# pmeletis/IV2019-boosting-semantic-segmentation-with-weak-labels

Hardware: NVIDIA B200
Metric: train_images_per_s (higher is better)
Workload: dtype bf16

## Files before the change

iv2019-boosting-semantic-segmentation-with-weak-labels_b200/csrc/conv_igemm_sm100.cu:

```cuda
#include <cuda.h>

#include <cstdlib>
#include <map>
#include <mutex>
#include <tuple>
#include <vector>

#include "common.cuh"
#include "tc_sm100.cuh"

namespace wlseg {

int check_conv_params(const wlseg_conv_params* p);
int conv_fprop_direct(const wlseg_conv_params* p, const void* x, const void* w, void* y, const float* scale,
                      const float* shift, const void* residual, cudaStream_t s);

constexpr int kBM = 128;
constexpr int kBK = 64;
constexpr int kUmmaK = 16;
constexpr int kEpiWarp0 = 4;
constexpr int kABytes = kBM * kBK * 2;
constexpr int kSmemBudget = 224 * 1024;

struct IgemmParams {
// ... 195 lines not shown
            const uint32_t lbar = mapa_shared(bar, 0);
            tma_load_4d_pair(a_dst, &prm.map_a, lbar, cc * kBK, q0 * prm.stride - prm.pad_left + s * prm.dilation,
                             p0 * prm.stride - prm.pad_top + r * prm.dilation, n);
            tma_load_3d_pair(b_dst, &prm.map_b, lbar, cc * kBK, tap, k0 + (int)rank * Cfg::kBRows);
          } else {
            mbar_arrive_expect_tx(bar, Cfg::kStageBytes);
            tma_load_4d(a_dst, &prm.map_a, bar, cc * kBK, q0 * prm.stride - prm.pad_left + s * prm.dilation,
                        p0 * prm.stride - prm.pad_top + r * prm.dilation, n);
            tma_load_3d(b_dst, &prm.map_b, bar, cc * kBK, tap, k0);
          }
          if (++stage == stages) { stage = 0; phase ^= 1; }
          if (++cc == prm.cchunks) {
            cc = 0; ++tap;
            if (++s == prm.S) { s = 0; ++r; }
          }
        }
      }
    }
  } else if (warp == 1) {
    if (kHalo && lane == 0) {
      constexpr uint32_t idesc = make_idesc(kBM, BN);
      mbar_wait(smem_u32(bfull_bar), 0);
      int iter = 0;
      for (int tile = unit0; tile < prm.units; tile += unit_step, ++iter) {
        const int acc = iter & 1, ab = iter & 1;
        const uint32_t ph = (iter >> 1) & 1;
        mbar_wait(smem_u32(tempty_bar + acc), ph ^ 1);
        mbar_wait(smem_u32(afull_bar + ab), ph);
        tc_fence_after();
        const uint32_t d_tmem = tmem_base + acc * BN;
        const uint32_t a_base = smem_u32(smem + ab * prm.halo_bytes);
        int r = 0, sx = 0;
        for (int kb = 0; kb < prm.num_kb; ++kb) {
          const uint64_t adesc = make_smem_desc_shifted(a_base + (uint32_t)(r * 2048 + sx * 128), (uint32_t)prm.halo_sbo);
          const uint64_t bdesc = make_smem_desc(smem_u32(halo_b + kb * Cfg::kBBytes));
#pragma unroll
          for (int k = 0; k < kBK / kUmmaK; ++k)
            umma_bf16(d_tmem, adesc + (uint64_t)(k * 2), bdesc + (uint64_t)(k * 2), idesc, (kb | k) != 0);
          if (++sx == prm.S) { sx = 0; ++r; }
        }
        umma_commit(smem_u32(aempty_bar + ab));
        umma_commit(smem_u32(tfull_bar + acc));
      }
    } else if (lane == 0 && rank == 0) {
      constexpr uint32_t idesc = make_idesc(kPair ? 2 * kBM : kBM, BN);
      int stage = 0;
      uint32_t phase = 0;
      int iter = 0;
      for (int tile = unit0; tile < prm.units; tile += unit_step, ++iter) {
        const int acc = iter & 1;
        const uint32_t acc_phase = (iter >> 1) & 1;
        mbar_wait(smem_u32(tempty_bar + acc), acc_phase ^ 1);
        tc_fence_after();
        const uint32_t d_tmem = tmem_base + acc * BN;
        for (int kb = 0; kb < prm.num_kb; ++kb) {
          mbar_wait(smem_u32(full_bar + stage), phase);
          tc_fence_after();
          const uint32_t a_addr = smem_u32(smem + stage * Cfg::kStageBytes);
          const uint64_t adesc = make_smem_desc(a_addr);
          const uint64_t bdesc = make_smem_desc(a_addr + kABytes);
#pragma unroll
          for (int k = 0; k < kBK / kUmmaK; ++k) {
            if (kPair) umma_bf16_pair(d_tmem, adesc + (uint64_t)(k * 2), bdesc + (uint64_t)(k * 2), idesc, (kb | k) != 0);
            else umma_bf16(d_tmem, adesc + (uint64_t)(k * 2), bdesc + (uint64_t)(k * 2), idesc, (kb | k) != 0);
          }
          if (kPair) umma_commit_pair(smem_u32(empty_bar + stage), 3); else umma_commit(smem_u32(empty_bar + stage));
          if (++stage == stages) { stage = 0; phase ^= 1; }
        }
        if (kPair) umma_commit_pair(smem_u32(tfull_bar + acc), 3); else umma_commit(smem_u32(tfull_bar + acc));
      }
    }
  } else if (warp >= kEpiWarp0) {
    const int ew = warp - kEpiWarp0;
    const int quarter = ew & 3;
    const int cgrp = ew >> 2;
    const int et = threadIdx.x - kEpiWarp0 * 32;
    const int row = quarter * 32 + lane;
    const int dy_ = row >> prm.tw_log2, dx_ = row & (TW - 1);
    const uint32_t lane_addr = tmem_base + ((uint32_t)(quarter * 32) << 16);
    auto release_acc = [&](int a) {
      if (kPair) mbar_arrive_cluster(mapa_shared(smem_u32(tempty_bar + a), 0));
      else mbar_arrive(smem_u32(tempty_bar + a));
    };
    int iter = 0;
    if constexpr (kTmaEpi) {
      const bool has_res = prm.res != nullptr;
      const bool has_stat = prm.bn_sum != nullptr;
      const uint32_t sw = (uint32_t)(lane & 7);
      const bool dbuf = has_res || prm.epi_db;
      const bool split = BN == kSubW && prm.epi_split != 0;
      uint8_t* wbuf = epi_smem + ((kHalo && !split) ? quarter : ew) * (kBnb ? 3 : (dbuf ? 2 : 1)) * kWarpBufBytes;
      const int st0 = split ? 0 : cgrp;
      const int st_step = split ? BN / kSubW : CG;
      const int tile0 = unit0 + (split ? cgrp * unit_step : 0);
      const int tile_step = split ? 2 * unit_step : unit_step;
      uint64_t* my_rfull = rfull_bar + 2 * ew;
      const int r0 = quarter * 32;
      const int dy0 = r0 >> prm.tw_log2, dx0 = r0 & (TW - 1);
      constexpr int kResPf = 4;
      struct ResCursor { int tile, st, cnt; };
      ResCursor ld = {tile0, st0, 0}, pf = {tile0, st0, 0};
      auto next_residual = [&](ResCursor& c, bool stage) {
        while (c.tile < prm.units) {
          int n, p0, q0, k0;
          decode_tile<BN, kPair>(prm, c.tile, rank, n, p0, q0, k0);
          if (c.st < num_subtiles<BN>(prm, k0)) {
            const int cx = (q0 + dx0) * prm.res_stride, cy = (p0 + dy0) * prm.res_stride;
            if (stage) {
              const uint32_t bar = smem_u32(my_rfull + (c.cnt & 1));
              mbar_arrive_expect_tx(bar, kWarpBufBytes);
              tma_load_4d(smem_u32(wbuf + (c.cnt & 1) * kWarpBufBytes), &prm.map_r, bar, k0 + c.st * kSubW, cx, cy, n);
            } else {
              tma_prefetch_4d(&prm.map_r, k0 + c.st * kSubW, cx, cy, n);
            }
            ++c.cnt;
            c.st += st_step;
            return;
          }
          c.st = st0;
          c.tile += tile_step;
        }
      };
      if (has_res && lane == 0) {
        for (int i = 0; i < kResPf; ++i) next_residual(pf, false);
        next_residual(ld, true);
      }
      constexpr int kSlots = (BN / kSubW + CG - 1) / CG;
      float a1x[kSlots], a1y[kSlots], a2x[kSlots], a2y[kSlots];
#pragma unroll
      for (int i = 0; i < kSlots; ++i) a1x[i] = a1y[i] = a2x[i] = a2y[i] = 0.f;
      int stat_k0 = -1;
      int cnt = 0;
      float bmx[kSlots], bmy[kSlots], bix[kSlots], biy[kSlots];
#pragma unroll
      for (int i = 0; i < kSlots; ++i) bmx[i] = bmy[i] = bix[i] = biy[i] = 0.f;
      uint2 mcur[kSlots], mnext[kSlots];
      auto load_mask = [&](int tile_, uint2 (&m)[kSlots]) {
#pragma unroll
        for (int i = 0; i < kSlots; ++i) m[i] = make_uint2(0xffffffffu, 0xffffffffu);
        if (prm.out_mask == nullptr || tile_ >= prm.units) return;
        int n_, p0_, q0_, k0_;
        decode_tile<BN, kPair>(prm, tile_, rank, n_, p0_, q0_, k0_);
        const bool ok = (p0_ + dy_ < prm.P) && (q0_ + dx_ < prm.Q) && (n_ < prm.N);
        const int nsub_ = num_subtiles<BN>(prm, k0_);
        const uint2* row = reinterpret_cast<const uint2*>(
            prm.out_mask + (((int64_t)n_ * prm.P + p0_ + dy_) * prm.Q + q0_ + dx_) * (prm.K >> 5) + (k0_ >> 5));
#pragma unroll
        for (int i = 0; i < kSlots; ++i) {
          const int st_ = st0 + i * st_step;
          m[i] = (ok && st_ < nsub_) ? __ldg(row + st_) : make_uint2(0u, 0u);
        }
      };
      load_mask(unit0, mnext);
      for (int tile = unit0; tile < prm.units; tile += unit_step, ++iter) {
        int n, p0, q0, k0;
        decode_tile<BN, kPair>(prm, tile, rank, n, p0, q0, k0);
        const bool valid = (p0 + dy_ < prm.P) && (q0 + dx_ < prm.Q) && (n < prm.N);
#pragma unroll
        for (int i = 0; i < kSlots; ++i) mcur[i] = mnext[i];
        load_mask(tile + unit_step, mnext);
        const int acc = iter & 1;
        const uint32_t acc_phase = (iter >> 1) & 1;
        const int nsub = num_subtiles<BN>(prm, k0);
        if (has_stat) {
          if (stat_k0 >= 0 && k0 != stat_k0) __trap();
          if constexpr (kBnb) {
            if (stat_k0 < 0) {
#pragma unroll
              for (int i = 0; i < kSlots; ++i) {
                const int c = k0 + (st0 + i * st_step) * kSubW + 2 * lane;
                if (c + 1 < prm.K) {
                  bmx[i] = __ldg(prm.bnb_mean + c); bmy[i] = __ldg(prm.bnb_mean + c + 1);
                  bix[i] = __ldg(prm.bnb_invstd + c); biy[i] = __ldg(prm.bnb_invstd + c + 1);
                }
              }
            }
          }
          stat_k0 = k0;
        }
        mbar_wait(smem_u32(tfull_bar + acc), acc_phase);
        tc_fence_after();
        const bool idle = split ? ((iter & 1) != cgrp) : (cgrp >= nsub);
        if (idle) {
          tc_fence_before();
          __syncwarp();
          if (lane == 0) release_acc(acc);
        }
#pragma unroll
        for (int slot = 0; slot < kSlots; ++slot) {
          const int st = st0 + slot * st_step;
          if (st >= nsub || idle) break;
          if constexpr (kBnb) {
            uint8_t* zb = wbuf + (cnt & 1) * kWarpBufBytes;
            uint8_t* ob = wbuf + 2 * kWarpBufBytes;
            if (lane == 0) {
              bulk_wait_read<0>();
              next_residual(ld, true);
              next_residual(pf, false);
            }
            __syncwarp();
            mbar_wait(smem_u32(my_rfull + (cnt & 1)), (uint32_t)((cnt >> 1) & 1));
#pragma unroll
            for (int half = 0; half < 2; ++half) {
              const int col = st * kSubW + half * 32;
              uint32_t v[32];
              tmem_ld<32>(lane_addr + (uint32_t)(acc * BN + col), v);
              tmem_ld_wait();
              if (half == 1 && st + CG >= nsub) {
                tc_fence_before();
                __syncwarp();
                if (lane == 0) release_acc(acc);
              }
              float f[32];
#pragma unroll
              for (int j = 0; j < 32; ++j) f[j] = valid ? __uint_as_float(v[j]) : 0.f;
              uint4 raw[4];
#pragma unroll
              for (int g = 0; g < 4; ++g)
                raw[g] = *reinterpret_cast<const uint4*>(zb + lane * 128 + ((((uint32_t)(half * 4 + g)) ^ sw) << 4));
              const float4* sc4 = reinterpret_cast<const float4*>(prm.bnb_scale + k0 + col);
              const float4* sh4 = reinterpret_cast<const float4*>(prm.bnb_shift + k0 + col);
              uint4 outv[4];
#pragma unroll
              for (int g = 0; g < 4; ++g) {
                const __nv_bfloat162* hz = reinterpret_cast<const __nv_bfloat162*>(&raw[g]);
                __nv_bfloat162* ho = reinterpret_cast<__nv_bfloat162*>(&outv[g]);
                const float4 sca = __ldg(sc4 + 2 * g), scb = __ldg(sc4 + 2 * g + 1);
                const float4 sha = __ldg(sh4 + 2 * g), shb = __ldg(sh4 + 2 * g + 1);
                const float scs[8] = {sca.x, sca.y, sca.z, sca.w, scb.x, scb.y, scb.z, scb.w};
                const float shs[8] = {sha.x, sha.y, sha.z, sha.w, shb.x, shb.y, shb.z, shb.w};
#pragma unroll
                for (int e = 0; e < 4; ++e) {
                  const float2 zz = __bfloat1622float2(hz[e]);
                  const float gx = fmaf(zz.x, scs[2 * e], shs[2 * e]) > 0.f ? f[g * 8 + 2 * e] : 0.f;
                  const float gy = fmaf(zz.y, scs[2 * e + 1], shs[2 * e + 1]) > 0.f ? f[g * 8 + 2 * e + 1] : 0.f;
                  ho[e] = __floats2bfloat162_rn(gx, gy);
                }
              }
#pragma unroll
              for (int g = 0; g < 4; ++g)
                *reinterpret_cast<uint4*>(ob + lane * 128 + ((((uint32_t)(half * 4 + g)) ^ sw) << 4)) = outv[g];
            }
            fence_async_smem();
            __syncwarp();
            if (lane == 0) {
              tma_store_4d(&prm.map_y, smem_u32(ob), k0 + st * kSubW, q0 + dx0, p0 + dy0, n);
              bulk_commit();
            }
            {
              const uint32_t coff = (uint32_t)((lane & 3) << 2);
              float s0x = 0.f, s0y = 0.f, s1x = 0.f, s1y = 0.f;
              const float mx = bmx[slot], my = bmy[slot], ix = bix[slot], iy = biy[slot];
#pragma unroll
              for (int r = 0; r < 32; ++r) {
                const uint32_t o = (uint32_t)(r * 128) + ((((uint32_t)(lane >> 2)) ^ (uint32_t)(r & 7)) << 4) + coff;
                const float2 g2 = __bfloat1622float2(*reinterpret_cast<const __nv_bfloat162*>(ob + o));
                const float2 z2 = __bfloat1622float2(*reinterpret_cast<const __nv_bfloat162*>(zb + o));
                s0x += g2.x * (z2.x - mx) * ix; s0y += g2.y * (z2.y - my) * iy;
                s1x += g2.x; s1y += g2.y;
              }
              a1x[slot] += s0x; a1y[slot] += s0y; a2x[slot] += s1x; a2y[slot] += s1y;
            }
            __syncwarp();
            ++cnt;
            continue;
          }
          uint8_t* buf = wbuf + (dbuf ? (cnt & 1) * kWarpBufBytes : 0);
          const bool mid = has_res && prm.res_mid;
          if (lane == 0 && !mid) {
            if (!has_res && dbuf) bulk_wait_read<1>(); else bulk_wait_read<0>();
            if (has_res) {
              next_residual(ld, true);
              next_residual(pf, false);
            }
          }
          __syncwarp();
          if (has_res && !mid) mbar_wait(smem_u32(my_rfull + (cnt & 1)), (uint32_t)((cnt >> 1) & 1));
          uint8_t* myrow = buf + lane * 128;
#pragma unroll
          for (int half = 0; half < 2; ++half) {
            const int col = st * kSubW + half * 32;
            if (mid && half == 1) {
              if (lane == 0) {
                bulk_wait_read<0>();
                next_residual(ld, true);
                next_residual(pf, false);
              }
              __syncwarp();
            }
            const uint32_t mword = half == 0 ? mcur[slot].x : mcur[slot].y;
            uint32_t v[32];
            tmem_ld<32>(lane_addr + (uint32_t)(acc * BN + col), v);
            tmem_ld_wait();
            if (half == 1 && st + CG >= nsub) {
              tc_fence_before();
              __syncwarp();
              if (lane == 0) release_acc(acc);
            }
            float f[32];
#pragma unroll
            for (int j = 0; j < 32; ++j) f[j] = __uint_as_float(v[j]);
            if (prm.scale != nullptr) {
              const float4* sc4 = reinterpret_cast<const float4*>(prm.scale + k0 + col);
              const float4* sh4 = reinterpret_cast<const float4*>(prm.shift + k0 + col);
#pragma unroll
              for (int g = 0; g < 8; ++g) {
                const float4 sc = __ldg(sc4 + g);
                const float4 sh = __ldg(sh4 + g);
                f[g * 4 + 0] = fmaf(f[g * 4 + 0], sc.x, sh.x);
                f[g * 4 + 1] = fmaf(f[g * 4 + 1], sc.y, sh.y);
                f[g * 4 + 2] = fmaf(f[g * 4 + 2], sc.z, sh.z);
                f[g * 4 + 3] = fmaf(f[g * 4 + 3], sc.w, sh.w);
              }
            }
            uint4* slot4[4];
#pragma unroll
            for (int g = 0; g < 4; ++g)
              slot4[g] = reinterpret_cast<uint4*>(myrow + ((((uint32_t)(half * 4 + g)) ^ sw) << 4));
            if (mid && half == 0) mbar_wait(smem_u32(my_rfull + (cnt & 1)), (uint32_t)((cnt >> 1) & 1));
            if (has_res) {
              uint4 raw[4];
#pragma unroll
              for (int g = 0; g < 4; ++g) raw[g] = *slot4[g];
#pragma unroll
              for (int g = 0; g < 4; ++g) {
                const __nv_bfloat162* h = reinterpret_cast<const __nv_bfloat162*>(&raw[g]);
#pragma unroll
                for (int e = 0; e < 4; ++e) {
                  const float2 t = __bfloat1622float2(h[e]);
                  f[g * 8 + 2 * e] += t.x;
                  f[g * 8 + 2 * e + 1] += t.y;
                }
              }
            }
            if (prm.out_mask != nullptr) {
#pragma unroll
              for (int j = 0; j < 32; ++j) f[j] = ((mword >> j) & 1u) ? f[j] : 0.f;
            }
            if (has_stat && !valid) {
#pragma unroll
              for (int j = 0; j < 32; ++j) f[j] = 0.f;
            }
            uint4 outv[4];
            if (prm.relu) {
#pragma unroll
              for (int g = 0; g < 4; ++g) {
                __nv_bfloat162* ho = reinterpret_cast<__nv_bfloat162*>(&outv[g]);
#pragma unroll
                for (int e = 0; e < 4; ++e) {
                  uint32_t packed;
                  asm("cvt.rn.relu.bf16x2.f32 %0, %1, %2;" : "=r"(packed) : "f"(f[g * 8 + 2 * e + 1]), "f"(f[g * 8 + 2 * e]));
                  reinterpret_cast<uint32_t*>(ho)[e] = packed;
                }
              }
            } else {
#pragma unroll
              for (int g = 0; g < 4; ++g) {
                __nv_bfloat162* ho = reinterpret_cast<__nv_bfloat162*>(&outv[g]);
#pragma unroll
                for (int e = 0; e < 4; ++e) ho[e] = __floats2bfloat162_rn(f[g * 8 + 2 * e], f[g * 8 + 2 * e + 1]);
              }
            }
#pragma unroll
            for (int g = 0; g < 4; ++g) *slot4[g] = outv[g];
          }
          fence_async_smem();
          __syncwarp();
          if (lane == 0) {
            tma_store_4d(&prm.map_y, smem_u32(buf), k0 + st * kSubW, q0 + dx0, p0 + dy0, n);
            bulk_commit();
          }
          if (has_stat) {
            const uint8_t* base = buf + ((lane & 3) << 2);
            float s1x = 0.f, s1y = 0.f, s2x = 0.f, s2y = 0.f;
#pragma unroll
            for (int r = 0; r < 32; ++r) {
              const __nv_bfloat162 h = *reinterpret_cast<const __nv_bfloat162*>(
                  base + r * 128 + ((((uint32_t)(lane >> 2)) ^ (uint32_t)(r & 7)) << 4));
              const float2 t = __bfloat1622float2(h);
              s1x += t.x; s1y += t.y;
              s2x = fmaf(t.x, t.x, s2x); s2y = fmaf(t.y, t.y, s2y);
            }
            a1x[slot] += s1x; a1y[slot] += s1y; a2x[slot] += s2x; a2y[slot] += s2y;
          }
          ++cnt;
        }
      }
      if (has_stat) {
        constexpr int kBufsPerWarp = kBnb ? 3 : 0;
        const int nbuf = kBufsPerWarp ? kBufsPerWarp : (dbuf ? 2 : 1);
        if (lane == 0) bulk_wait_read<0>();
        __syncwarp();
        float* park = reinterpret_cast<float*>(wbuf);
#pragma unroll
        for (int i = 0; i < kSlots; ++i) {
          if (kHalo && !split && cgrp != 0) break;
          park[(i * 2 + 0) * kSubW + 2 * lane] = a1x[i]; park[(i * 2 + 0) * kSubW + 2 * lane + 1] = a1y[i];
          park[(i * 2 + 1) * kSubW + 2 * lane] = a2x[i]; park[(i * 2 + 1) * kSubW + 2 * lane + 1] = a2y[i];
        }
        epi_barrier<32 * EW>();
        if (stat_k0 >= 0) {
          for (int j = et; j < BN; j += 32 * EW) {
            if (stat_k0 + j < prm.K) {
              const int st = j / kSubW, ch = j % kSubW;
              const int cg = split ? 0 : st % CG, i = split ? 0 : st / CG;
              float t1 = 0.f, t2 = 0.f;
              for (int g2 = 0; g2 < (split ? CG : 1); ++g2) {
#pragma unroll
                for (int q4 = 0; q4 < 4; ++q4) {
                  const float* src = reinterpret_cast<const float*>(epi_smem + (q4 + 4 * (cg + g2)) * nbuf * kWarpBufBytes);
                  t1 += src[(i * 2 + 0) * kSubW + ch];
                  t2 += src[(i * 2 + 1) * kSubW + ch];
                }
              }
              atomicAdd(prm.bn_sum + stat_k0 + j, (double)t1);
              atomicAdd(prm.bn_sqsum + stat_k0 + j, (double)t2);
            }
          }
        }
      }
      if constexpr (!kBnb) {
        if (has_stat && prm.fin.counter != nullptr) {
          uint32_t* s_last = tmem_slot + 1;
          __threadfence();
          epi_barrier<32 * EW>();
          if (et == 0) *s_last = (atomicAdd(prm.fin.counter, 1u) == gridDim.x - 1) ? 1u : 0u;
          epi_barrier<32 * EW>();
          if (*s_last != 0u) {
            __threadfence();
            const double nn = (double)prm.fin.count;
            for (int c = et; c < prm.K; c += 32 * EW) {
              const double m = __ldcg(prm.bn_sum + c) / nn;
              double var = __ldcg(prm.bn_sqsum + c) / nn - m * m;
              if (var < 0.0) var = 0.0;
              const float mf = (float)m, vf = (float)var;
              const float inv = rsqrtf(vf + prm.fin.eps);
              const float sc = prm.fin.gamma[c] * inv;
              prm.fin.scale[c] = sc;
              prm.fin.shift[c] = prm.fin.beta[c] - mf * sc;
              prm.fin.saved_mean[c] = mf;
              prm.fin.saved_invstd[c] = inv;
              if (prm.fin.moving_mean != nullptr) {
                const float unbiased = prm.fin.moving_var_factor >= 0.f
                                           ? vf * prm.fin.moving_var_factor
                                           : (prm.fin.count > 1 ? (float)(var * (nn / (nn - 1.0))) : vf);
                prm.fin.moving_mean[c] -= (1.0f - prm.fin.decay) * (prm.fin.moving_mean[c] - mf);
                prm.fin.moving_var[c] -= (1.0f - prm.fin.decay) * (prm.fin.moving_var[c] - unbiased);
              }
            }
            if (et == 0) *prm.fin.counter = 0u;
          }
        }
      }
      if (lane == 0) bulk_wait_all();
    } else {
      for (int tile = unit0; tile < prm.units; tile += unit_step, ++iter) {
        int n, p0, q0, k0;
        decode_tile<BN, kPair>(prm, tile, rank, n, p0, q0, k0);
        const int q = q0 + dx_;
        const int p = p0 + dy_;
        const bool valid = (p < prm.P) && (q < prm.Q) && (n < prm.N);
        const int acc = iter & 1;
        const uint32_t acc_phase = (iter >> 1) & 1;
        mbar_wait(smem_u32(tfull_bar + acc), acc_phase);
        tc_fence_after();
        const int64_t opix = ((int64_t)n * prm.P + p) * prm.Q + q;
        TY* yrow = reinterpret_cast<TY*>(prm.y) + opix * prm.y_pitch;
        const __nv_bfloat16* rrow = nullptr;
        if (prm.res != nullptr && valid)
          rrow = reinterpret_cast<const __nv_bfloat16*>(prm.res) +
                 (((int64_t)n * prm.res_H + (int64_t)p * prm.res_stride) * prm.res_W + (int64_t)q * prm.res_stride) *
                     prm.res_pitch;
#pragma unroll 1
        for (int ch = cgrp; ch < BN / 32; ch += CG) {
          const int kbase = k0 + ch * 32;
          if (kbase >= prm.K) break;
          uint32_t v[32];
          tmem_ld<32>(lane_addr + (uint32_t)(acc * BN + ch * 32), v);
          tmem_ld_wait();
          float f[32];
#pragma unroll
// ... 301 lines not shown
      uint64_t dims[4] = {(uint64_t)p->C, (uint64_t)p->W, (uint64_t)p->H, (uint64_t)p->N};
      uint64_t strides[3] = {(uint64_t)p->x_pitch * 2, (uint64_t)p->x_pitch * 2 * p->W, (uint64_t)p->x_pitch * 2 * p->W * p->H};
      uint32_t box[4] = {(uint32_t)kBK, 16, (uint32_t)prm.halo_rows, 1};
      uint32_t estr[4] = {1, 1, 1, 1};
      if (int e = encode_tensor_map(&prm.map_ah, x, 2, 4, dims, strides, box, estr, 4)) return e;
    }
  }
  {
    uint64_t dims[3] = {(uint64_t)p->C, (uint64_t)(p->R * p->S), (uint64_t)p->K};
    uint64_t strides[2] = {(uint64_t)p->C * 2, (uint64_t)p->C * 2 * p->R * p->S};
    uint32_t box[3] = {(uint32_t)kBK, 1, (uint32_t)(use_pair ? BN / 2 : BN)};
    uint32_t estr[3] = {1, 1, 1};
    if (int e = encode_tensor_map(&prm.map_b, w, 2, 3, dims, strides, box, estr, 1)) return e;
  }
  if (tma_epi) {
    {
      uint64_t dims[4] = {(uint64_t)p->K, (uint64_t)p->Q, (uint64_t)p->P, (uint64_t)p->N};
      uint64_t strides[3] = {(uint64_t)p->y_pitch * 2, (uint64_t)p->y_pitch * 2 * p->Q,
                             (uint64_t)p->y_pitch * 2 * p->Q * p->P};
      uint32_t box[4] = {(uint32_t)kSubW, (uint32_t)bw, (uint32_t)bh, 1};
      uint32_t estr[4] = {1, 1, 1, 1};
      if (int e = encode_tensor_map(&prm.map_y, y, 2, 4, dims, strides, box, estr, 2)) return e;
    }
    if (residual != nullptr) {
      const int rs = p->res_stride;
      uint64_t dims[4] = {(uint64_t)p->K, (uint64_t)p->res_W, (uint64_t)p->res_H, (uint64_t)p->N};
      uint64_t strides[3] = {(uint64_t)p->res_pitch * 2, (uint64_t)p->res_pitch * 2 * p->res_W,
                             (uint64_t)p->res_pitch * 2 * p->res_W * p->res_H};
      uint32_t box[4] = {(uint32_t)kSubW, (uint32_t)(bw * rs), (uint32_t)(bh * rs), 1};
      uint32_t estr[4] = {1, (uint32_t)rs, (uint32_t)rs, 1};
      if (int e = encode_tensor_map(&prm.map_r, residual, 2, 4, dims, strides, box, estr, 3)) return e;
    }
  }
  prm.y = y; prm.scale = scale; prm.shift = shift; prm.res = residual;
  prm.bn_sum = bn_sum; prm.bn_sqsum = bn_sqsum;
  prm.out_mask = out_mask;
  prm.bnb_scale = prm.bnb_shift = prm.bnb_mean = prm.bnb_invstd = nullptr;
  prm.fin = wlseg_bn_finalize_args{};
  if (fin != nullptr) {
    WLSEG_CHECK_ARG(tma_epi && bn_sum != nullptr && bnb == nullptr && !pdl_enabled(),
                    "conv_fprop_bn: needs the staged bf16 epilogue (K %% 64 == 0, aligned y) and no programmatic launches");
    prm.fin = *fin;
  }
  if (bnb != nullptr) {
    prm.bnb_scale = bnb->scale; prm.bnb_shift = bnb->shift; prm.bnb_mean = bnb->mean; prm.bnb_invstd = bnb->invstd;
  }
  WLSEG_CHECK_ARG(out_mask == nullptr || (tma_epi && p->K % 32 == 0 && (((uintptr_t)out_mask) & 3) == 0),
                  "conv_fprop_masked: needs the staged bf16 epilogue (K %% 64 == 0, aligned tensors)");
  prm.N = p->N; prm.P = p->P; prm.Q = p->Q; prm.K = p->K; prm.C = p->C;
  prm.R = p->R; prm.S = p->S; prm.stride = p->stride; prm.dilation = p->dilation;
  prm.pad_top = p->pad_top; prm.pad_left = p->pad_left;
  prm.y_pitch = p->y_pitch; prm.res_pitch = p->res_pitch; prm.res_stride = p->res_stride;
  prm.res_H = p->res_H; prm.res_W = p->res_W;
  prm.relu = p->relu;
  prm.reverse = p->reverse ? 1 : 0;
  prm.tw_log2 = tw_log2;
  prm.tiles_w = (int)ceil_div(p->Q, TW);
  prm.tiles_h = (int)ceil_div(p->P, TH);
  prm.n_tiles = (int)ceil_div(p->K, BN);
  const int64_t total = (int64_t)p->N * prm.tiles_h * prm.tiles_w * prm.n_tiles;
  WLSEG_CHECK_ARG(total < ((int64_t)1 << 31), "conv(tcgen05): too many tiles");
  prm.total_tiles = (int)total;
  prm.m_tiles = (int)(total / prm.n_tiles);
  prm.fd_n_tiles = make_fastdiv((uint32_t)prm.n_tiles);
  prm.fd_tiles_w = make_fastdiv((uint32_t)prm.tiles_w);
  prm.fd_tiles_h = make_fastdiv((uint32_t)prm.tiles_h);
  prm.units = prm.total_tiles;
  prm.cchunks = (int)ceil_div(p->C, kBK);
  prm.num_kb = p->R * p->S * prm.cchunks;
#define WLSEG_IGEMM_CASE(bn)                                                          \
  case bn:                                                                            \
    if (f32out) return launch_igemm<bn, float, false>(prm, s);                        \
    if (bn >= kSubW && tma_epi) return launch_igemm<bn, __nv_bfloat16, (bn >= kSubW)>(prm, s); \
    return launch_igemm<bn, __nv_bfloat16, false>(prm, s);
  if (use_halo) {
    if (bnb != nullptr) return launch_igemm_ew<64, __nv_bfloat16, true, 8, false, true, true>(prm, s);
    return launch_igemm_ew<64, __nv_bfloat16, true, 8, false, false, true>(prm, s);
  }
  if (bnb != nullptr) {
    if (BN == 256) return launch_igemm_ew<256, __nv_bfloat16, true, 8, true, true>(prm, s);
    if (BN == 128) return launch_igemm_ew<128, __nv_bfloat16, true, 8, false, true>(prm, s);
    return launch_igemm_ew<64, __nv_bfloat16, true, 8, false, true>(prm, s);
  }
  if (use_pair) return launch_igemm_ew<256, __nv_bfloat16, true, 8, true>(prm, s);
  switch (BN) {
    WLSEG_IGEMM_CASE(32)
    WLSEG_IGEMM_CASE(64)
    WLSEG_IGEMM_CASE(128)
    WLSEG_IGEMM_CASE(256)
  }
#undef WLSEG_IGEMM_CASE
  WLSEG_CHECK_ARG(false, "conv(tcgen05): internal tile selection error");
}

}

using namespace wlseg;

extern "C" int wlseg_conv2d_tcgen05_supported(const wlseg_conv_params* p) {
  if (p == nullptr) return 0;
  return igemm_supported(p) ? 1 : 0;
}

extern "C" int wlseg_conv2d_fprop_masked(const wlseg_conv_params* p, const void* x, const void* w, void* y,
                                         const void* residual, const uint8_t* out_mask, wlseg_stream_t stream) {
  if (int e = check_conv_params(p)) return e;
  if (p->N == 0) return 0;
  WLSEG_CHECK_ARG(x && w && y && out_mask, "conv_fprop_masked: null pointer");
  WLSEG_CHECK_ARG(igemm_supported(p) && p->y_dtype == WLSEG_BF16 && p->relu == 0,
                  "conv_fprop_masked: tcgen05 bf16 configurations without ReLU only");
  if (residual != nullptr)
    WLSEG_CHECK_ARG(p->res_stride > 0 && p->res_pitch >= p->K && (p->P - 1) * p->res_stride < p->res_H &&
                        (p->Q - 1) * p->res_stride < p->res_W,
                    "conv_fprop_masked: residual geometry inconsistent");
  return conv_fprop_igemm(p, x, w, y, nullptr, nullptr, residual, nullptr, nullptr, (cudaStream_t)stream,
                          reinterpret_cast<const uint32_t*>(out_mask));
}

extern "C" int wlseg_conv2d_fprop_bnbwd(const wlseg_conv_params* p, const void* x, const void* w, void* y, const void* z,
                                        const float* scale, const float* shift, const float* mean, const float* invstd,
                                        double* dgamma, double* dbeta, wlseg_stream_t stream) {
  if (int e = check_conv_params(p)) return e;
  if (p->N == 0) return 0;
  WLSEG_CHECK_ARG(x && w && y && z && scale && shift && mean && invstd && dgamma && dbeta, "conv_fprop_bnbwd: null pointer");
  WLSEG_CHECK_ARG(igemm_supported(p) && p->y_dtype == WLSEG_BF16 && p->relu == 0 && p->K % 64 == 0,
                  "conv_fprop_bnbwd: tcgen05 bf16 configurations with K %% 64 == 0 and without ReLU only");
  WLSEG_CHECK_ARG(p->res_stride == 1 && p->res_pitch >= p->K && p->res_H == p->P && p->res_W == p->Q,
                  "conv_fprop_bnbwd: z must have the output's shape (res_* fields of the parameters describe it)");
  WLSEG_CHECK_ARG(((((uintptr_t)scale) | ((uintptr_t)shift)) & 15) == 0, "conv_fprop_bnbwd: scale / shift must be 16-byte aligned");
  const BnbArgs bnb = {scale, shift, mean, invstd};
  return conv_fprop_igemm(p, x, w, y, nullptr, nullptr, z, dgamma, dbeta, (cudaStream_t)stream, nullptr, &bnb);
}

extern "C" int wlseg_conv2d_fprop_bn(const wlseg_conv_params* p, const void* x, const void* w, void* y, double* bn_sum,
                                     double* bn_sqsum, const wlseg_bn_finalize_args* fin, wlseg_stream_t stream) {
  if (int e = check_conv_params(p)) return e;
  if (p->N == 0) return 0;
  WLSEG_CHECK_ARG(x && w && y && bn_sum && bn_sqsum && fin, "conv_fprop_bn: null pointer");
  WLSEG_CHECK_ARG(fin->count > 0 && fin->gamma && fin->beta && fin->scale && fin->shift && fin->saved_mean &&
                      fin->saved_invstd && fin->counter && ((fin->moving_mean == nullptr) == (fin->moving_var == nullptr)),
                  "conv_fprop_bn: incomplete wlseg_bn_finalize_args");
  WLSEG_CHECK_ARG(igemm_supported(p) && p->y_dtype == WLSEG_BF16 && p->relu == 0 && p->K % 64 == 0,
                  "conv_fprop_bn: tcgen05 bf16 configurations with K %% 64 == 0 and without ReLU only");
  return conv_fprop_igemm(p, x, w, y, nullptr, nullptr, nullptr, bn_sum, bn_sqsum, (cudaStream_t)stream, nullptr, nullptr, fin);
}

extern "C" int wlseg_conv2d_fprop(const wlseg_conv_params* p, const void* x, const void* w, void* y,
                                  const float* scale, const float* shift, const void* residual, double* bn_sum,
                                  double* bn_sqsum, wlseg_stream_t stream) {
  if (int e = check_conv_params(p)) return e;
  if (p->N == 0) return 0;
  WLSEG_CHECK_ARG(x && w && y, "conv_fprop: null pointer");
  WLSEG_CHECK_ARG((scale == nullptr) == (shift == nullptr), "conv_fprop: scale and shift must come together");
  WLSEG_CHECK_ARG((bn_sum == nullptr) == (bn_sqsum == nullptr), "conv_fprop: bn_sum and bn_sqsum must come together");
  if (residual != nullptr)
    WLSEG_CHECK_ARG(p->res_stride > 0 && p->res_pitch >= p->K && (p->P - 1) * p->res_stride < p->res_H &&
                        (p->Q - 1) * p->res_stride < p->res_W,
                    "conv_fprop: residual geometry inconsistent");
  int algo = p->algo;
  if (algo == WLSEG_ALGO_AUTO) algo = igemm_supported(p) ? WLSEG_ALGO_TCGEN05 : WLSEG_ALGO_DIRECT;
  if (algo == WLSEG_ALGO_TCGEN05) {
    WLSEG_CHECK_ARG(igemm_supported(p), "conv_fprop: configuration not covered by the tcgen05 kernel");
    return conv_fprop_igemm(p, x, w, y, scale, shift, residual, bn_sum, bn_sqsum, (cudaStream_t)stream);
  }
  WLSEG_CHECK_ARG(algo == WLSEG_ALGO_DIRECT, "conv_fprop: unknown algo %d", algo);
  WLSEG_CHECK_ARG(bn_sum == nullptr, "conv_fprop(direct): fused BN statistics are not available; call wlseg_bn_stats");
  return conv_fprop_direct(p, x, w, y, scale, shift, residual, (cudaStream_t)stream);
// ... 2 lines not shown
```

iv2019-boosting-semantic-segmentation-with-weak-labels_b200/csrc/tc_sm100.cuh:

```cuda
#pragma once

#include <cuda.h>

#include "common.cuh"

namespace wlseg {

__device__ __forceinline__ uint32_t smem_u32(const void* p) { return (uint32_t)__cvta_generic_to_shared(p); }

__device__ __forceinline__ void mbar_init(uint32_t bar, uint32_t count) {
  asm volatile("mbarrier.init.shared::cta.b64 [%0], %1;" ::"r"(bar), "r"(count) : "memory");
}
__device__ __forceinline__ void mbar_arrive_expect_tx(uint32_t bar, uint32_t bytes) {
  asm volatile("mbarrier.arrive.expect_tx.shared::cta.b64 _, [%0], %1;" ::"r"(bar), "r"(bytes) : "memory");
}
__device__ __forceinline__ void mbar_arrive(uint32_t bar) {
  asm volatile("mbarrier.arrive.shared::cta.b64 _, [%0];" ::"r"(bar) : "memory");
}
__device__ __forceinline__ bool mbar_try_wait(uint32_t bar, uint32_t parity) {
  uint32_t ok;
  asm volatile(
      "{\n\t.reg .pred p;\n\t"
      "mbarrier.try_wait.parity.shared::cta.b64 p, [%1], %2;\n\t"
      "selp.u32 %0, 1, 0, p;\n\t}"
// ... 12 lines not shown
__device__ __forceinline__ void tc_fence_before() { asm volatile("tcgen05.fence::before_thread_sync;" ::: "memory"); }
__device__ __forceinline__ void tc_fence_after() { asm volatile("tcgen05.fence::after_thread_sync;" ::: "memory"); }

__device__ __forceinline__ void tma_load_4d(uint32_t dst, const CUtensorMap* map, uint32_t bar, int c0, int c1, int c2,
                                            int c3) {
  asm volatile(
      "cp.async.bulk.tensor.4d.shared::cluster.global.mbarrier::complete_tx::bytes [%0], [%1, {%3, %4, %5, %6}], [%2];"
      ::"r"(dst), "l"((uint64_t)map), "r"(bar), "r"(c0), "r"(c1), "r"(c2), "r"(c3)
      : "memory");
}
__device__ __forceinline__ void tma_load_3d(uint32_t dst, const CUtensorMap* map, uint32_t bar, int c0, int c1, int c2) {
  asm volatile(
      "cp.async.bulk.tensor.3d.shared::cluster.global.mbarrier::complete_tx::bytes [%0], [%1, {%3, %4, %5}], [%2];"
      ::"r"(dst), "l"((uint64_t)map), "r"(bar), "r"(c0), "r"(c1), "r"(c2)
      : "memory");
}
__device__ __forceinline__ void tma_prefetch_4d(const CUtensorMap* map, int c0, int c1, int c2, int c3) {
  asm volatile("cp.async.bulk.prefetch.tensor.4d.L2.global [%0, {%1, %2, %3, %4}];"
               ::"l"((uint64_t)map), "r"(c0), "r"(c1), "r"(c2), "r"(c3)
               : "memory");
}
__device__ __forceinline__ void tma_store_4d(const CUtensorMap* map, uint32_t src, int c0, int c1, int c2, int c3) {
  asm volatile("cp.async.bulk.tensor.4d.global.shared::cta.bulk_group [%0, {%2, %3, %4, %5}], [%1];"
               ::"l"((uint64_t)map), "r"(src), "r"(c0), "r"(c1), "r"(c2), "r"(c3)
               : "memory");
}
__device__ __forceinline__ void bulk_commit() { asm volatile("cp.async.bulk.commit_group;" ::: "memory"); }
template <int N>
__device__ __forceinline__ void bulk_wait_read() { asm volatile("cp.async.bulk.wait_group.read %0;" ::"n"(N) : "memory"); }
__device__ __forceinline__ void bulk_wait_all() { asm volatile("cp.async.bulk.wait_group 0;" ::: "memory"); }
__device__ __forceinline__ void fence_async_smem() { asm volatile("fence.proxy.async.shared::cta;" ::: "memory"); }
template <int kThreads>
__device__ __forceinline__ void epi_barrier() { asm volatile("bar.sync 1, %0;" ::"n"(kThreads) : "memory"); }

__device__ __forceinline__ void tma_prefetch_desc(const CUtensorMap* map) {
  asm volatile("prefetch.tensormap [%0];" ::"l"((uint64_t)map) : "memory");
}

__device__ __forceinline__ void tmem_alloc(uint32_t smem_dst, uint32_t ncols) {
  asm volatile("tcgen05.alloc.cta_group::1.sync.aligned.shared::cta.b32 [%0], %1;" ::"r"(smem_dst), "r"(ncols) : "memory");
  asm volatile("tcgen05.relinquish_alloc_permit.cta_group::1.sync.aligned;" ::: "memory");
}
__device__ __forceinline__ void tmem_dealloc(uint32_t taddr, uint32_t ncols) {
  asm volatile("tcgen05.dealloc.cta_group::1.sync.aligned.b32 %0, %1;" ::"r"(taddr), "r"(ncols) : "memory");
}
__device__ __forceinline__ void umma_bf16(uint32_t d_tmem, uint64_t adesc, uint64_t bdesc, uint32_t idesc,
                                          uint32_t accumulate) {
  asm volatile(
      "{\n\t.reg .pred p;\n\t"
      "setp.ne.b32 p, %4, 0;\n\t"
      "tcgen05.mma.cta_group::1.kind::f16 [%0], %1, %2, %3, p;\n\t}"
      ::"r"(d_tmem), "l"(adesc), "l"(bdesc), "r"(idesc), "r"(accumulate)
      : "memory");
}
__device__ __forceinline__ void umma_commit(uint32_t bar) {
  asm volatile("tcgen05.commit.cta_group::1.mbarrier::arrive::one.shared::cluster.b64 [%0];" ::"r"(bar) : "memory");
}
__device__ __forceinline__ void tmem_ld32(uint32_t taddr, uint32_t (&v)[32]) {
  asm volatile(
      "tcgen05.ld.sync.aligned.32x32b.x32.b32 "
      "{%0, %1, %2, %3, %4, %5, %6, %7, %8, %9, %10, %11, %12, %13, %14, %15, "
      "%16, %17, %18, %19, %20, %21, %22, %23, %24, %25, %26, %27, %28, %29, %30, %31}, [%32];"
      : "=r"(v[0]), "=r"(v[1]), "=r"(v[2]), "=r"(v[3]), "=r"(v[4]), "=r"(v[5]), "=r"(v[6]), "=r"(v[7]), "=r"(v[8]),
        "=r"(v[9]), "=r"(v[10]), "=r"(v[11]), "=r"(v[12]), "=r"(v[13]), "=r"(v[14]), "=r"(v[15]), "=r"(v[16]),
        "=r"(v[17]), "=r"(v[18]), "=r"(v[19]), "=r"(v[20]), "=r"(v[21]), "=r"(v[22]), "=r"(v[23]), "=r"(v[24]),
        "=r"(v[25]), "=r"(v[26]), "=r"(v[27]), "=r"(v[28]), "=r"(v[29]), "=r"(v[30]), "=r"(v[31])
      : "r"(taddr)
      : "memory");
}
__device__ __forceinline__ void tmem_ld16(uint32_t taddr, uint32_t (&v)[16]) {
  asm volatile(
      "tcgen05.ld.sync.aligned.32x32b.x16.b32 "
      "{%0, %1, %2, %3, %4, %5, %6, %7, %8, %9, %10, %11, %12, %13, %14, %15}, [%16];"
      : "=r"(v[0]), "=r"(v[1]), "=r"(v[2]), "=r"(v[3]), "=r"(v[4]), "=r"(v[5]), "=r"(v[6]), "=r"(v[7]), "=r"(v[8]),
        "=r"(v[9]), "=r"(v[10]), "=r"(v[11]), "=r"(v[12]), "=r"(v[13]), "=r"(v[14]), "=r"(v[15])
      : "r"(taddr)
      : "memory");
}
template <int kCols> __device__ __forceinline__ void tmem_ld(uint32_t taddr, uint32_t (&v)[kCols]);
template <> __device__ __forceinline__ void tmem_ld<32>(uint32_t taddr, uint32_t (&v)[32]) { tmem_ld32(taddr, v); }
template <> __device__ __forceinline__ void tmem_ld<16>(uint32_t taddr, uint32_t (&v)[16]) { tmem_ld16(taddr, v); }
__device__ __forceinline__ void tmem_ld_wait() { asm volatile("tcgen05.wait::ld.sync.aligned;" ::: "memory"); }

__device__ __forceinline__ uint32_t cluster_ctarank() {
  uint32_t r;
  asm volatile("mov.u32 %0, %%cluster_ctarank;" : "=r"(r));
  return r;
}
__device__ __forceinline__ void cluster_sync() {
  asm volatile("barrier.cluster.arrive.release.aligned;\n\tbarrier.cluster.wait.acquire.aligned;" ::: "memory");
}
__device__ __forceinline__ void cluster_sync_relaxed() {
  asm volatile("barrier.cluster.arrive.relaxed.aligned;\n\tbarrier.cluster.wait.aligned;" ::: "memory");
}
__device__ __forceinline__ uint32_t mapa_shared(uint32_t addr, uint32_t rank) {
  uint32_t r;
  asm volatile("mapa.shared::cluster.u32 %0, %1, %2;" : "=r"(r) : "r"(addr), "r"(rank));
  return r;
}
__device__ __forceinline__ void mbar_arrive_cluster(uint32_t cluster_bar) {
  asm volatile("mbarrier.arrive.shared::cluster.b64 _, [%0];" ::"r"(cluster_bar) : "memory");
}
__device__ __forceinline__ void tma_load_4d_pair(uint32_t dst, const CUtensorMap* map, uint32_t cluster_bar, int c0, int c1,
                                                 int c2, int c3) {
  asm volatile(
      "cp.async.bulk.tensor.4d.cta_group::2.shared::cluster.global.mbarrier::complete_tx::bytes [%0], [%1, {%3, %4, %5, %6}], [%2];"
      ::"r"(dst), "l"((uint64_t)map), "r"(cluster_bar), "r"(c0), "r"(c1), "r"(c2), "r"(c3)
      : "memory");
}
__device__ __forceinline__ void tma_load_3d_pair(uint32_t dst, const CUtensorMap* map, uint32_t cluster_bar, int c0, int c1,
                                                 int c2) {
  asm volatile(
      "cp.async.bulk.tensor.3d.cta_group::2.shared::cluster.global.mbarrier::complete_tx::bytes [%0], [%1, {%3, %4, %5}], [%2];"
      ::"r"(dst), "l"((uint64_t)map), "r"(cluster_bar), "r"(c0), "r"(c1), "r"(c2)
      : "memory");
}
__device__ __forceinline__ void tmem_alloc_pair(uint32_t smem_dst, uint32_t ncols) {
  asm volatile("tcgen05.alloc.cta_group::2.sync.aligned.shared::cta.b32 [%0], %1;" ::"r"(smem_dst), "r"(ncols) : "memory");
  asm volatile("tcgen05.relinquish_alloc_permit.cta_group::2.sync.aligned;" ::: "memory");
}
__device__ __forceinline__ void tmem_dealloc_pair(uint32_t taddr, uint32_t ncols) {
  asm volatile("tcgen05.dealloc.cta_group::2.sync.aligned.b32 %0, %1;" ::"r"(taddr), "r"(ncols) : "memory");
}
__device__ __forceinline__ void umma_bf16_pair(uint32_t d_tmem, uint64_t adesc, uint64_t bdesc, uint32_t idesc,
                                               uint32_t accumulate) {
  asm volatile(
      "{\n\t.reg .pred p;\n\t"
      "setp.ne.b32 p, %4, 0;\n\t"
      "tcgen05.mma.cta_group::2.kind::f16 [%0], %1, %2, %3, p;\n\t}"
      ::"r"(d_tmem), "l"(adesc), "l"(bdesc), "r"(idesc), "r"(accumulate)
      : "memory");
}
__device__ __forceinline__ void umma_commit_pair(uint32_t bar, uint16_t cta_mask) {
  asm volatile("tcgen05.commit.cta_group::2.mbarrier::arrive::one.shared::cluster.multicast::cluster.b64 [%0], %1;"
               ::"r"(bar), "h"(cta_mask)
               : "memory");
}

__device__ __forceinline__ uint64_t make_smem_desc(uint32_t saddr) {
  uint64_t d = 0;
  d |= (uint64_t)((saddr & 0x3FFFFu) >> 4);
  d |= (uint64_t)1 << 16;
  d |= (uint64_t)(1024 >> 4) << 32;
  d |= (uint64_t)1 << 46;
  d |= (uint64_t)2 << 61;
  return d;
}
__device__ __forceinline__ uint64_t make_smem_desc_shifted(uint32_t saddr, uint32_t sbo) {
  uint64_t d = 0;
  d |= (uint64_t)((saddr & 0x3FFFFu) >> 4);
  d |= (uint64_t)1 << 16;
  d |= (uint64_t)(sbo >> 4) << 32;
  d |= (uint64_t)1 << 46;
  d |= (uint64_t)2 << 61;
  return d;
}
__host__ __device__ constexpr uint32_t make_idesc(int m, int n) {
  return (1u << 4) | (1u << 7) | (1u << 10) | ((uint32_t)(n >> 3) << 17) | ((uint32_t)(m >> 4) << 24);
}

}
```

Baseline: 382.3.

## Vectorize conv epilogue with packed float2 math and batch TMEM loads

```diff
diff --git a/iv2019-boosting-semantic-segmentation-with-weak-labels_b200/csrc/conv_igemm_sm100.cu b/iv2019-boosting-semantic-segmentation-with-weak-labels_b200/csrc/conv_igemm_sm100.cu
--- a/iv2019-boosting-semantic-segmentation-with-weak-labels_b200/csrc/conv_igemm_sm100.cu
+++ b/iv2019-boosting-semantic-segmentation-with-weak-labels_b200/csrc/conv_igemm_sm100.cu
@@ -301,6 +301,25 @@
       if (kPair) mbar_arrive_cluster(mapa_shared(smem_u32(tempty_bar + a), 0));
       else mbar_arrive(smem_u32(tempty_bar + a));
     };
+    constexpr bool kWideLd = EW <= 8;
+    auto hand_back = [&](int a, int st_, int nsub_) {
+      if (st_ + CG >= nsub_) {
+        tc_fence_before();
+        __syncwarp();
+        if (lane == 0) release_acc(a);
+      }
+    };
+    auto load_subtile = [&](uint32_t (&v)[2][32], int a, int st_, int nsub_) {
+      tmem_ld<32>(lane_addr + (uint32_t)(a * BN + st_ * kSubW), v[0]);
+      tmem_ld<32>(lane_addr + (uint32_t)(a * BN + st_ * kSubW + 32), v[1]);
+      tmem_ld_wait();
+      hand_back(a, st_, nsub_);
+    };
+    auto load_half = [&](uint32_t (&v)[32], int a, int st_, int nsub_, int half) {
+      tmem_ld<32>(lane_addr + (uint32_t)(a * BN + st_ * kSubW + half * 32), v);
+      tmem_ld_wait();
+      if (half == 1) hand_back(a, st_, nsub_);
+    };
     int iter = 0;
     if constexpr (kTmaEpi) {
       const bool has_res = prm.res != nullptr;
@@ -345,14 +364,14 @@
         next_residual(ld, true);
       }
       constexpr int kSlots = (BN / kSubW + CG - 1) / CG;
-      float a1x[kSlots], a1y[kSlots], a2x[kSlots], a2y[kSlots];
-#pragma unroll
-      for (int i = 0; i < kSlots; ++i) a1x[i] = a1y[i] = a2x[i] = a2y[i] = 0.f;
+      float2 a1[kSlots], a2[kSlots];
+#pragma unroll
+      for (int i = 0; i < kSlots; ++i) a1[i] = a2[i] = make_float2(0.f, 0.f);
       int stat_k0 = -1;
       int cnt = 0;
-      float bmx[kSlots], bmy[kSlots], bix[kSlots], biy[kSlots];
-#pragma unroll
-      for (int i = 0; i < kSlots; ++i) bmx[i] = bmy[i] = bix[i] = biy[i] = 0.f;
+      float2 bnm[kSlots], bi[kSlots];
+#pragma unroll
+      for (int i = 0; i < kSlots; ++i) { bnm[i] = make_float2(-0.f, -0.f); bi[i] = make_float2(0.f, 0.f); }
       uint2 mcur[kSlots], mnext[kSlots];
       auto load_mask = [&](int tile_, uint2 (&m)[kSlots]) {
 #pragma unroll
@@ -389,8 +408,8 @@
               for (int i = 0; i < kSlots; ++i) {
                 const int c = k0 + (st0 + i * st_step) * kSubW + 2 * lane;
                 if (c + 1 < prm.K) {
-                  bmx[i] = __ldg(prm.bnb_mean + c); bmy[i] = __ldg(prm.bnb_mean + c + 1);
-                  bix[i] = __ldg(prm.bnb_invstd + c); biy[i] = __ldg(prm.bnb_invstd + c + 1);
+                  bnm[i] = make_float2(-__ldg(prm.bnb_mean + c), -__ldg(prm.bnb_mean + c + 1));
+                  bi[i] = make_float2(__ldg(prm.bnb_invstd + c), __ldg(prm.bnb_invstd + c + 1));
                 }
               }
             }
@@ -419,20 +438,16 @@
             }
             __syncwarp();
             mbar_wait(smem_u32(my_rfull + (cnt & 1)), (uint32_t)((cnt >> 1) & 1));
+            uint32_t v[2][32];
+            if constexpr (kWideLd) load_subtile(v, acc, st, nsub);
 #pragma unroll
             for (int half = 0; half < 2; ++half) {
               const int col = st * kSubW + half * 32;
-              uint32_t v[32];
-              tmem_ld<32>(lane_addr + (uint32_t)(acc * BN + col), v);
-              tmem_ld_wait();
-              if (half == 1 && st + CG >= nsub) {
-                tc_fence_before();
-                __syncwarp();
-                if (lane == 0) release_acc(acc);
-              }
-              float f[32];
-#pragma unroll
-              for (int j = 0; j < 32; ++j) f[j] = valid ? __uint_as_float(v[j]) : 0.f;
+              if constexpr (!kWideLd) load_half(v[half], acc, st, nsub, half);
+              if (!valid) {
+#pragma unroll
+                for (int j = 0; j < 32; ++j) v[half][j] = 0u;
+              }
               uint4 raw[4];
 #pragma unroll
               for (int g = 0; g < 4; ++g)
@@ -442,18 +457,20 @@
               uint4 outv[4];
 #pragma unroll
               for (int g = 0; g < 4; ++g) {
-                const __nv_bfloat162* hz = reinterpret_cast<const __nv_bfloat162*>(&raw[g]);
-                __nv_bfloat162* ho = reinterpret_cast<__nv_bfloat162*>(&outv[g]);
+                const uint32_t* wz = &raw[g].x;
+                uint32_t* wo = &outv[g].x;
                 const float4 sca = __ldg(sc4 + 2 * g), scb = __ldg(sc4 + 2 * g + 1);
                 const float4 sha = __ldg(sh4 + 2 * g), shb = __ldg(sh4 + 2 * g + 1);
-                const float scs[8] = {sca.x, sca.y, sca.z, sca.w, scb.x, scb.y, scb.z, scb.w};
-                const float shs[8] = {sha.x, sha.y, sha.z, sha.w, shb.x, shb.y, shb.z, shb.w};
+                const float2 scs[4] = {{sca.x, sca.y}, {sca.z, sca.w}, {scb.x, scb.y}, {scb.z, scb.w}};
+                const float2 shs[4] = {{sha.x, sha.y}, {sha.z, sha.w}, {shb.x, shb.y}, {shb.z, shb.w}};
 #pragma unroll
                 for (int e = 0; e < 4; ++e) {
-                  const float2 zz = __bfloat1622float2(hz[e]);
-                  const float gx = fmaf(zz.x, scs[2 * e], shs[2 * e]) > 0.f ? f[g * 8 + 2 * e] : 0.f;
-                  const float gy = fmaf(zz.y, scs[2 * e + 1], shs[2 * e + 1]) > 0.f ? f[g * 8 + 2 * e + 1] : 0.f;
-                  ho[e] = __floats2bfloat162_rn(gx, gy);
+                  const float2 a = __ffma2_rn(bf16x2_to_float2(wz[e]), scs[e], shs[e]);
+                  const int j = g * 8 + 2 * e;
+                  const float gx = a.x > 0.f ? __uint_as_float(v[half][j]) : 0.f;
+                  const float gy = a.y > 0.f ? __uint_as_float(v[half][j + 1]) : 0.f;
+                  const __nv_bfloat162 h = __floats2bfloat162_rn(gx, gy);
+                  wo[e] = *reinterpret_cast<const uint32_t*>(&h);
                 }
               }
 #pragma unroll
@@ -468,17 +485,16 @@
             }
             {
               const uint32_t coff = (uint32_t)((lane & 3) << 2);
-              float s0x = 0.f, s0y = 0.f, s1x = 0.f, s1y = 0.f;
-              const float mx = bmx[slot], my = bmy[slot], ix = bix[slot], iy = biy[slot];
+              float2 s0 = make_float2(0.f, 0.f), s1 = make_float2(0.f, 0.f);
 #pragma unroll
               for (int r = 0; r < 32; ++r) {
                 const uint32_t o = (uint32_t)(r * 128) + ((((uint32_t)(lane >> 2)) ^ (uint32_t)(r & 7)) << 4) + coff;
-                const float2 g2 = __bfloat1622float2(*reinterpret_cast<const __nv_bfloat162*>(ob + o));
-                const float2 z2 = __bfloat1622float2(*reinterpret_cast<const __nv_bfloat162*>(zb + o));
-                s0x += g2.x * (z2.x - mx) * ix; s0y += g2.y * (z2.y - my) * iy;
-                s1x += g2.x; s1y += g2.y;
-              }
-              a1x[slot] += s0x; a1y[slot] += s0y; a2x[slot] += s1x; a2y[slot] += s1y;
+                const float2 g2 = bf16x2_to_float2(*reinterpret_cast<const uint32_t*>(ob + o));
+                const float2 z2 = bf16x2_to_float2(*reinterpret_cast<const uint32_t*>(zb + o));
+                s0 = __ffma2_rn(__fmul2_rn(g2, __fadd2_rn(z2, bnm[slot])), bi[slot], s0);
+                s1 = __fadd2_rn(s1, g2);
+              }
+              a1[slot] = __fadd2_rn(a1[slot], s0); a2[slot] = __fadd2_rn(a2[slot], s1);
             }
             __syncwarp();
             ++cnt;
@@ -496,9 +512,12 @@
           __syncwarp();
           if (has_res && !mid) mbar_wait(smem_u32(my_rfull + (cnt & 1)), (uint32_t)((cnt >> 1) & 1));
           uint8_t* myrow = buf + lane * 128;
+          uint32_t v[2][32];
+          if constexpr (kWideLd) load_subtile(v, acc, st, nsub);
 #pragma unroll
           for (int half = 0; half < 2; ++half) {
             const int col = st * kSubW + half * 32;
+            if constexpr (!kWideLd) load_half(v[half], acc, st, nsub, half);
             if (mid && half == 1) {
               if (lane == 0) {
                 bulk_wait_read<0>();
@@ -507,18 +526,9 @@
               }
               __syncwarp();
             }
-            const uint32_t mword = half == 0 ? mcur[slot].x : mcur[slot].y;
-            uint32_t v[32];
-            tmem_ld<32>(lane_addr + (uint32_t)(acc * BN + col), v);
-            tmem_ld_wait();
-            if (half == 1 && st + CG >= nsub) {
-              tc_fence_before();
-              __syncwarp();
-              if (lane == 0) release_acc(acc);
-            }
-            float f[32];
-#pragma unroll
-            for (int j = 0; j < 32; ++j) f[j] = __uint_as_float(v[j]);
+            float2 f[16];
+#pragma unroll
+            for (int e = 0; e < 16; ++e) f[e] = u32x2_as_float2(v[half][2 * e], v[half][2 * e + 1]);
             if (prm.scale != nullptr) {
               const float4* sc4 = reinterpret_cast<const float4*>(prm.scale + k0 + col);
               const float4* sh4 = reinterpret_cast<const float4*>(prm.shift + k0 + col);
@@ -526,10 +536,8 @@
               for (int g = 0; g < 8; ++g) {
                 const float4 sc = __ldg(sc4 + g);
                 const float4 sh = __ldg(sh4 + g);
-                f[g * 4 + 0] = fmaf(f[g * 4 + 0], sc.x, sh.x);
-                f[g * 4 + 1] = fmaf(f[g * 4 + 1], sc.y, sh.y);
-                f[g * 4 + 2] = fmaf(f[g * 4 + 2], sc.z, sh.z);
-                f[g * 4 + 3] = fmaf(f[g * 4 + 3], sc.w, sh.w);
+                f[2 * g] = __ffma2_rn(f[2 * g], make_float2(sc.x, sc.y), make_float2(sh.x, sh.y));
+                f[2 * g + 1] = __ffma2_rn(f[2 * g + 1], make_float2(sc.z, sc.w), make_float2(sh.z, sh.w));
               }
             }
             uint4* slot4[4];
@@ -543,41 +551,38 @@
               for (int g = 0; g < 4; ++g) raw[g] = *slot4[g];
 #pragma unroll
               for (int g = 0; g < 4; ++g) {
-                const __nv_bfloat162* h = reinterpret_cast<const __nv_bfloat162*>(&raw[g]);
-#pragma unroll
-                for (int e = 0; e < 4; ++e) {
-                  const float2 t = __bfloat1622float2(h[e]);
-                  f[g * 8 + 2 * e] += t.x;
-                  f[g * 8 + 2 * e + 1] += t.y;
-                }
+                const uint32_t* w = &raw[g].x;
+#pragma unroll
+                for (int e = 0; e < 4; ++e) f[g * 4 + e] = __fadd2_rn(f[g * 4 + e], bf16x2_to_float2(w[e]));
               }
             }
             if (prm.out_mask != nullptr) {
-#pragma unroll
-              for (int j = 0; j < 32; ++j) f[j] = ((mword >> j) & 1u) ? f[j] : 0.f;
+              const uint32_t mword = half == 0 ? mcur[slot].x : mcur[slot].y;
+#pragma unroll
+              for (int e = 0; e < 16; ++e) {
+                if (!((mword >> (2 * e)) & 1u)) f[e].x = 0.f;
+                if (!((mword >> (2 * e + 1)) & 1u)) f[e].y = 0.f;
+              }
             }
             if (has_stat && !valid) {
 #pragma unroll
-              for (int j = 0; j < 32; ++j) f[j] = 0.f;
+              for (int e = 0; e < 16; ++e) f[e] = make_float2(0.f, 0.f);
             }
             uint4 outv[4];
             if (prm.relu) {
 #pragma unroll
               for (int g = 0; g < 4; ++g) {
-                __nv_bfloat162* ho = reinterpret_cast<__nv_bfloat162*>(&outv[g]);
 #pragma unroll
                 for (int e = 0; e < 4; ++e) {
-                  uint32_t packed;
-                  asm("cvt.rn.relu.bf16x2.f32 %0, %1, %2;" : "=r"(packed) : "f"(f[g * 8 + 2 * e + 1]), "f"(f[g * 8 + 2 * e]));
-                  reinterpret_cast<uint32_t*>(ho)[e] = packed;
+                  asm("cvt.rn.relu.bf16x2.f32 %0, %1, %2;" : "=r"((&outv[g].x)[e]) : "f"(f[g * 4 + e].y), "f"(f[g * 4 + e].x));
                 }
               }
             } else {
 #pragma unroll
               for (int g = 0; g < 4; ++g) {
-                __nv_bfloat162* ho = reinterpret_cast<__nv_bfloat162*>(&outv[g]);
-#pragma unroll
-                for (int e = 0; e < 4; ++e) ho[e] = __floats2bfloat162_rn(f[g * 8 + 2 * e], f[g * 8 + 2 * e + 1]);
+#pragma unroll
+                for (int e = 0; e < 4; ++e)
+                  asm("cvt.rn.bf16x2.f32 %0, %1, %2;" : "=r"((&outv[g].x)[e]) : "f"(f[g * 4 + e].y), "f"(f[g * 4 + e].x));
               }
             }
 #pragma unroll
@@ -591,16 +596,15 @@
           }
           if (has_stat) {
             const uint8_t* base = buf + ((lane & 3) << 2);
-            float s1x = 0.f, s1y = 0.f, s2x = 0.f, s2y = 0.f;
+            float2 s1 = make_float2(0.f, 0.f), s2 = make_float2(0.f, 0.f);
 #pragma unroll
             for (int r = 0; r < 32; ++r) {
-              const __nv_bfloat162 h = *reinterpret_cast<const __nv_bfloat162*>(
-                  base + r * 128 + ((((uint32_t)(lane >> 2)) ^ (uint32_t)(r & 7)) << 4));
-              const float2 t = __bfloat1622float2(h);
-              s1x += t.x; s1y += t.y;
-              s2x = fmaf(t.x, t.x, s2x); s2y = fmaf(t.y, t.y, s2y);
-            }
-            a1x[slot] += s1x; a1y[slot] += s1y; a2x[slot] += s2x; a2y[slot] += s2y;
+              const float2 t = bf16x2_to_float2(*reinterpret_cast<const uint32_t*>(
+                  base + r * 128 + ((((uint32_t)(lane >> 2)) ^ (uint32_t)(r & 7)) << 4)));
+              s1 = __fadd2_rn(s1, t);
+              s2 = __ffma2_rn(t, t, s2);
+            }
+            a1[slot] = __fadd2_rn(a1[slot], s1); a2[slot] = __fadd2_rn(a2[slot], s2);
           }
           ++cnt;
         }
@@ -614,8 +618,8 @@
 #pragma unroll
         for (int i = 0; i < kSlots; ++i) {
           if (kHalo && !split && cgrp != 0) break;
-          park[(i * 2 + 0) * kSubW + 2 * lane] = a1x[i]; park[(i * 2 + 0) * kSubW + 2 * lane + 1] = a1y[i];
-          park[(i * 2 + 1) * kSubW + 2 * lane] = a2x[i]; park[(i * 2 + 1) * kSubW + 2 * lane + 1] = a2y[i];
+          *reinterpret_cast<float2*>(park + (i * 2 + 0) * kSubW + 2 * lane) = a1[i];
+          *reinterpret_cast<float2*>(park + (i * 2 + 1) * kSubW + 2 * lane) = a2[i];
         }
         epi_barrier<32 * EW>();
         if (stat_k0 >= 0) {
@@ -1083,7 +1087,12 @@
     if (BN == 128) return launch_igemm_ew<128, __nv_bfloat16, true, 8, false, true>(prm, s);
     return launch_igemm_ew<64, __nv_bfloat16, true, 8, false, true>(prm, s);
   }
-  if (use_pair) return launch_igemm_ew<256, __nv_bfloat16, true, 8, true>(prm, s);
+  const bool wide_epi = BN == 256 && tma_epi && residual == nullptr && p->R * p->S * (int)ceil_div(p->C, kBK) <= 4;
+  if (use_pair) {
+    if (wide_epi) return launch_igemm_ew<256, __nv_bfloat16, true, 16, true>(prm, s);
+    return launch_igemm_ew<256, __nv_bfloat16, true, 8, true>(prm, s);
+  }
+  if (wide_epi) return launch_igemm_ew<256, __nv_bfloat16, true, 16>(prm, s);
   switch (BN) {
     WLSEG_IGEMM_CASE(32)
     WLSEG_IGEMM_CASE(64)
diff --git a/iv2019-boosting-semantic-segmentation-with-weak-labels_b200/csrc/tc_sm100.cuh b/iv2019-boosting-semantic-segmentation-with-weak-labels_b200/csrc/tc_sm100.cuh
--- a/iv2019-boosting-semantic-segmentation-with-weak-labels_b200/csrc/tc_sm100.cuh
+++ b/iv2019-boosting-semantic-segmentation-with-weak-labels_b200/csrc/tc_sm100.cuh
@@ -118,6 +118,13 @@
 template <> __device__ __forceinline__ void tmem_ld<16>(uint32_t taddr, uint32_t (&v)[16]) { tmem_ld16(taddr, v); }
 __device__ __forceinline__ void tmem_ld_wait() { asm volatile("tcgen05.wait::ld.sync.aligned;" ::: "memory"); }
 
+__device__ __forceinline__ float2 u32x2_as_float2(uint32_t x, uint32_t y) {
+  return make_float2(__uint_as_float(x), __uint_as_float(y));
+}
+__device__ __forceinline__ float2 bf16x2_to_float2(uint32_t w) {
+  return make_float2(__uint_as_float(w << 16), __uint_as_float(w & 0xffff0000u));
+}
+
 __device__ __forceinline__ uint32_t cluster_ctarank() {
   uint32_t r;
   asm volatile("mov.u32 %0, %%cluster_ctarank;" : "=r"(r));
```

Result: no change. 385.1, median of 6 (+0.7%).
